# nvpro-samples/vk_gltf_renderer

Measured on AMD Instinct MI355X. Metric: Msamples/s (and ms/frame @ fixed spp) 1080p & 4K, 1/2/4/8 MI355X, higher is better.
Workload: dtype f32

## Files before the change

### vk_gltf_renderer_amd/csrc/device/mi_pt_api.hip

```cpp
#include <hip/hip_runtime.h>

#include <algorithm>
#include <chrono>
#include <cstdlib>
#include <cmath>
#include <cstdio>
#include <cstring>
#include <memory>
#include <string>
#include <vector>

#include "mi_pt.h"
#include "bvh_refit.h"
#include "material_patch.h"
#include "pt_build.h"
#include "pt_bvh.h"
#include "pt_deform.h"
#include "pt_kernels.h"

namespace {

thread_local std::string g_lastError;

int fail(int code, const std::string& msg)
// ... 129 lines not shown
  DevBuf<pt::DevPrim>         prims;
  DevBuf<MiGltfLight>         lights;
  DevBuf<pt::DevTexture>      textures;
  DevBuf<uchar4>              texels;
  DevBuf<uint4>               texQuads;
  DevBuf<uint8_t>             geometry;
  DevBuf<uint8_t>             instFlags;
  DevBuf<float>               srgbLut;
  DevBuf<float4>              envPixels;
  DevBuf<MiEnvAccel>          envAccel;
  DevBuf<pt::DevAlphaTri>     alphaTris;
  DevBuf<pt::DevShadeTri>     shadeTris;
  float4*                     bvhNodes  = nullptr;
  uint4*                      bvh8Nodes = nullptr;
  DevBuf<float>               bvh8Planes;
  pt::DevTri*                 bvhTris   = nullptr;
  bool                        wide      = true;
  pt::DevScene                scene{};
  bool                        hasAlpha = false, hasAlphaTest = false, hasVolumeScatter = false, simpleMaterials = true, hasTransmissive = false;
  static constexpr int        FC_RING = 32;
  DevBuf<pt::DevScene>        sceneDev;
  bool                        sceneDevDirty = true;
  DevBuf<pt::FrameConsts>     fcRing;
  DevBuf<pt::SkyPrecomp>      skyPre;
  MiSkyPhysicalParameters     skyPreFor{};
  bool                        skyPreValid = false;
  pt::FrameConsts*            fcHost = nullptr;
  hipEvent_t                  fcDone[FC_RING] = {};
  unsigned                    fcCursor = 0;
  MiPtStats                   staticStats{};
// ... 383 lines not shown
  }
  pt->lastUpdate = MI_PT_ACCEL_LAST_BUILD;
  if(rc != MI_PT_OK)
    dropAcceleration(pt);
  return rc;
}
void dropAcceleration(MiPt* pt)
{
  {
    const std::string why = g_lastError;
    releaseRefitData(pt);
    if(pt->bvhNodes) (void)hipFree(pt->bvhNodes);
    if(pt->bvhTris) (void)hipFree(pt->bvhTris);
    if(pt->bvh8Nodes) (void)hipFree(pt->bvh8Nodes);
    pt->bvhNodes = nullptr; pt->bvhTris = nullptr; pt->bvh8Nodes = nullptr;
    pt->bvh8Planes.release(); pt->shadeTris.release(); pt->alphaTris.release();
    pt::DevScene& S = pt->scene;
    S.bvhNodes = nullptr; S.bvh8Nodes = nullptr; S.tris = nullptr; S.bvh8Planes = nullptr; S.shadeTris = nullptr; S.alphaTris = nullptr;
    S.numTris = 0; S.bvh8NumNodes = 0; S.bvhRoot = pt::BVH_EMPTY;
    pt->staticStats.bvhNodeCount = pt->staticStats.bvhTriangleCount = 0;
    pt->sceneDevDirty = true;
    g_lastError = why;
  }
}
std::vector<uint8_t> instanceFlags(MiPt* pt)
{
  const int            numNodes = int(pt->hostNodes.size()), numMaterials = int(pt->matInstFlags.size());
  std::vector<uint8_t> flags(size_t(std::max(numNodes, 1)), 0);
  pt->hasAlpha = pt->hasAlphaTest = pt->hasTransmissive = pt->hasVolumeScatter = false;
  pt->simpleMaterials = true;
  for(int n = 0; n < numNodes; ++n)
  {
    const MiGltfRenderNode& rn = pt->hostNodes[size_t(n)];
// ... 136 lines not shown
      (void)hipFree(pt->bvhNodes);
      (void)hipFree(pt->bvhTris);
      pt->bvhNodes  = nullptr;
      pt->bvhTris   = b8.tris;
      pt->bvh8Nodes = b8.nodes;
      pt->scene.bvhRoot = 0;
      pt->scene.bvh8NumNodes = int(b8.numNodes);
      pt->staticStats.bvhNodeCount = b8.numNodes;
      pt->staticStats.bvhNodeBytes = 80;
      if(!pt->sw.noPlanes)
      {
        HIP_TRY(pt->bvh8Planes.alloc(size_t(b8.numNodes) * 48));
        pt::launchBvh8Planes(b8.nodes, b8.numNodes, pt->bvh8Planes.ptr, nullptr);
        HIP_TRY(hipGetLastError());
      }
      if(b8.slotBox && b8.nodeBox)
      {
        HIP_TRY(pt->refitBuiltBox.alloc(b8.numTris));
        HIP_TRY(hipMemcpy(pt->refitBuiltBox.ptr, b8.slotBox, sizeof(pt::RefitBox) * size_t(b8.numTris), hipMemcpyDeviceToDevice));
        HIP_TRY(pt->refitSah.alloc(b8.numNodes));
        HIP_TRY(pt->refitSahPartial.alloc(pt::REFIT_SAH_PARTIALS + 1));
        HIP_TRY(pt->refitDirty.alloc(std::max<size_t>(pt->hostNodes.size(), 1)));
        pt::launchRefitLevels(b8.nodes, b8.levels, pt->refitSlotBox.ptr, pt->refitNodeBox.ptr, pt->refitSah.ptr, nullptr);
        if(pt->bvh8Planes.ptr)
          pt::launchBvh8Planes(b8.nodes, b8.numNodes, pt->bvh8Planes.ptr, nullptr);
        HIP_TRY(hipGetLastError());
        if(int rc = readSahCost(pt, pt->sahAtBuild))
          return rc;
        pt->sahNow      = pt->sahAtBuild;
        pt->refitLevels = b8.levels;
        pt->builtNodes  = pt->hostNodes;
        pt->primDirty.assign(pt->primTriangles.size(), 0);
        pt->primDeformed.assign(pt->primTriangles.size(), 0);
        pt->residentTree = resident;
        pt->hiddenTris   = resident ? hiddenTris : 0;
      }
      else
      {
        pt->refitSlotBox.release();
        pt->refitNodeBox.release();
      }
    }
  }
  if(resident && !pt->residentTree && hiddenTris > 0)
  {
    --pt->accelBuilds;
    return buildAccelerationOver(pt, false);
  }
  pt::DevScene& S = pt->scene;
  S.bvhNodes = pt->bvhNodes; S.bvh8Nodes = pt->bvh8Nodes; S.tris = pt->bvhTris;
  S.bvh8Planes = pt->bvh8Nodes ? pt->bvh8Planes.ptr : nullptr;
  S.shadeTris = nullptr;
  S.alphaTris = nullptr;
  if(S.numTris > 0)
  {
    HIP_TRY(pt->shadeTris.alloc(size_t(S.numTris)));
    pt::launchBuildShadeRecords(S, uint32_t(S.numTris), pt->shadeTris.ptr, nullptr);
    HIP_TRY(hipGetLastError());
    HIP_TRY(hipDeviceSynchronize());
    S.shadeTris = pt->shadeTris.ptr;
  }
  if(pt->hasAlpha && S.numTris > 0)
  {
    HIP_TRY(pt->alphaTris.alloc(size_t(S.numTris)));
    pt::launchBuildAlphaRecords(S, uint32_t(S.numTris), pt->alphaTris.ptr, nullptr);
    HIP_TRY(hipGetLastError());
    HIP_TRY(hipDeviceSynchronize());
    S.alphaTris = pt->alphaTris.ptr;
  }
  if(pt->residentTree && pt->hiddenTris > 0)
  {
    std::vector<uint8_t> dirty(std::max<size_t>(pt->hostNodes.size(), 1), pt::REFIT_CLEAN);
    for(size_t n = 0; n < pt->hostNodes.size(); ++n)
      if(!pt->hostVisible[n])
        dirty[n] = pt::REFIT_HIDDEN;
    HIP_TRY(hipMemcpy(pt->refitDirty.ptr, dirty.data(), dirty.size(), hipMemcpyHostToDevice));
    pt::launchRefitTris(pt->nodes.ptr, pt->prims.ptr, pt->instFlags.ptr, pt->refitDirty.ptr, pt->refitBuiltBox.ptr, pt->bvhTris, pt->refitSlotBox.ptr,
                        uint32_t(S.numTris), nullptr);
    pt::launchRefitLevels(pt->bvh8Nodes, pt->refitLevels, pt->refitSlotBox.ptr, pt->refitNodeBox.ptr, pt->refitSah.ptr, nullptr);
    if(pt->bvh8Planes.ptr)
      pt::launchBvh8Planes(pt->bvh8Nodes, uint32_t(S.bvh8NumNodes), pt->bvh8Planes.ptr, nullptr);
    HIP_TRY(hipGetLastError());
    if(int rc = readSahCost(pt, pt->sahNow))
      return rc;
    HIP_TRY(hipDeviceSynchronize());
  }
  pt->sceneDevDirty = true;
  return MI_PT_OK;
}

int refitAcceleration(MiPt* pt, const std::vector<uint8_t>& moved, const std::vector<uint8_t>* visWas = nullptr)
{
  static const bool    buildTiming = getenv("MI_PT_BUILD_TIMING") != nullptr;
  const auto           t0          = std::chrono::steady_clock::now();
  const size_t         numNodes = pt->hostNodes.size(), numPrims = pt->primTriangles.size();
  std::vector<uint8_t> dirty(std::max<size_t>(numNodes, 1), pt::REFIT_CLEAN);
// ... 25 lines not shown
    const bool home = memcmp(rn.objectToWorld, pt->builtNodes[n].objectToWorld, sizeof(float) * 32) == 0 && !(ownsPrim && pt->primDeformed[size_t(rn.renderPrimID)]);
    dirty[n]        = home ? pt::REFIT_HOME : pt::REFIT_MOVED;
    if(ownsPrim && (pt->hostVisible.empty() || pt->hostVisible[n]))
      movedTris += pt->primTriangles[size_t(rn.renderPrimID)];
  }
  const std::vector<uint8_t> flags = instanceFlags(pt);
  const int                  rc    = [&]() -> int {
    HIP_TRY(hipMemcpy(pt->nodes.ptr, pt->hostNodes.data(), sizeof(MiGltfRenderNode) * numNodes, hipMemcpyHostToDevice));
    HIP_TRY(hipMemcpy(pt->instFlags.ptr, flags.data(), flags.size(), hipMemcpyHostToDevice));
    HIP_TRY(hipMemcpy(pt->refitDirty.ptr, dirty.data(), dirty.size(), hipMemcpyHostToDevice));
    pt::launchRefitTris(pt->nodes.ptr, pt->prims.ptr, pt->instFlags.ptr, pt->refitDirty.ptr, pt->refitBuiltBox.ptr, pt->bvhTris, pt->refitSlotBox.ptr,
                        uint32_t(pt->scene.numTris), nullptr);
    pt::launchRefitLevels(pt->bvh8Nodes, pt->refitLevels, pt->refitSlotBox.ptr, pt->refitNodeBox.ptr, pt->refitSah.ptr, nullptr);
    if(pt->bvh8Planes.ptr)
      pt::launchBvh8Planes(pt->bvh8Nodes, uint32_t(pt->scene.bvh8NumNodes), pt->bvh8Planes.ptr, nullptr);
    HIP_TRY(hipGetLastError());
    if(int e = readSahCost(pt, pt->sahNow))
      return e;
    HIP_TRY(hipDeviceSynchronize());
    return MI_PT_OK;
  }();
  if(rc != MI_PT_OK)
  {
    dropAcceleration(pt);
    return rc;
  }
  std::fill(pt->primDirty.begin(), pt->primDirty.end(), uint8_t(0));
  pt->sceneDevDirty = true;
  if(buildTiming)
    fprintf(stderr, "[mi_pt build] %-28s %8.2f ms\n", "refit", std::chrono::duration<double, std::milli>(std::chrono::steady_clock::now() - t0).count());
// ... 484 lines not shown
    HIP_TRY(pt->coreTex.upload(core.data(), core.size()));
  }
  {
    float lut[256];
    for(int i = 0; i < 256; ++i)
    {
      float c = float(i) / 255.0f;
      lut[i]  = c <= 0.04045f ? c / 12.92f : std::pow((c + 0.055f) / 1.055f, 2.4f);
    }
    HIP_TRY(pt->srgbLut.upload(lut, 256));
  }
  phase("textures upload");

  pt::DevScene& S = pt->scene;
  S.materials = pt->materials.ptr; S.texInfos = pt->texInfos.ptr; S.nodes = pt->nodes.ptr; S.prims = pt->prims.ptr; S.lights = pt->lights.ptr;
  S.textures = pt->textures.ptr; S.texels = pt->texels.ptr; S.texQuads = pt->texQuads.ptr; S.envPixels = nullptr; S.envAccel = nullptr; S.bvhNodes = nullptr; S.bvh8Nodes = nullptr; S.bvh8Planes = nullptr; S.tris = nullptr;
  S.geomPool = reinterpret_cast<const float4*>(pt->geometry.ptr);
  S.texRefs = pt->texRefs.ptr; S.coreTex = reinterpret_cast<const uint4*>(pt->coreTex.ptr); S.alphaTris = nullptr; S.shadeTris = nullptr; S.srgbLut = pt->srgbLut.ptr; S.numMaterials = sd->numMaterials; S.numTextures = sd->numTextures;
  S.numLights = sd->numLights; S.numNodes = sd->numRenderNodes;
  S.envWidth = 0; S.envHeight = 0;
  S.packetInterval = pt->sw.packetInterval;
  S.shadowOctFlip  = pt->sw.shadowFarFirst ? 7u : 0u;
  if(int rc = buildAcceleration(pt.get()))
    return rc;
  phase("shade / alpha records");
  HIP_TRY(pt->stats.alloc(1));
  HIP_TRY(hipMemset(pt->stats.ptr, 0, sizeof(pt::StatCounters)));
  MiSkyPhysicalParameters s{};
  s.rgbUnitConversion[0] = s.rgbUnitConversion[1] = s.rgbUnitConversion[2] = 1.0f / 80000.0f;
  s.multiplier = 0.1f; s.haze = 0.1f; s.redblueshift = 0.1f; s.saturation = 1.0f; s.groundColor[0] = s.groundColor[1] = s.groundColor[2] = 0.4f;
  s.horizonBlur = 0.3f; s.sunDiskIntensity = 1.0f; s.sunDirection[0] = s.sunDirection[1] = s.sunDirection[2] = 0.5773502691896258f;
// ... 1235 lines not shown

void* mi_pt_tonemapped_device_ptr(MiPt* pt)
{
  return pt ? pt->tonemapped.ptr : nullptr;
}

int mi_pt_get_memory(MiPt* pt, MiPtMemory* out)
{
  if(!pt || !out)
    return fail(MI_PT_ERR_ARGUMENT, "mi_pt_get_memory: null argument");
  HIP_TRY(hipSetDevice(pt->device));
  auto bytes = [](const auto& b) { return uint64_t(b.count) * sizeof(*b.ptr); };
  const pt::DevScene& sc = pt->scene;
  uint64_t scene = bytes(pt->materials) + bytes(pt->texInfos) + bytes(pt->nodes) + bytes(pt->prims) + bytes(pt->lights) + bytes(pt->textures) + bytes(pt->texels) + bytes(pt->texQuads)
                   + bytes(pt->geometry) + bytes(pt->instFlags) + bytes(pt->srgbLut) + bytes(pt->envPixels) + bytes(pt->envAccel) + bytes(pt->alphaTris)
                   + bytes(pt->shadeTris) + bytes(pt->texRefs) + bytes(pt->coreTex) + bytes(pt->bvh8Planes) + bytes(pt->deformPool) + bytes(pt->deformTasks)
                   + bytes(pt->deformBlockTask) + bytes(pt->deformJoints) + bytes(pt->deformWeights) + refitBytes(pt) + bytes(pt->vmPrevPositions) + bytes(pt->vmPrims)
                   + bytes(pt->vmDeformIDs);
  scene += uint64_t(pt->staticStats.bvhNodeCount) * pt->staticStats.bvhNodeBytes + uint64_t(sc.numTris) * sizeof(pt::DevTri);
  const uint64_t pathState = bytes(pt->pathArrays) + bytes(pt->optThroughput) + bytes(pt->optMisc) + bytes(pt->optMedium) + bytes(pt->optPixelSum) + bytes(pt->optGuides)
                             + bytes(pt->optShadowAux2) + bytes(pt->queueMem) + bytes(pt->queuePayload) + bytes(pt->candPool) + bytes(pt->candLists);
  const uint64_t renderer = pathState + bytes(pt->firstHit) + bytes(pt->accumOwn)
                            + bytes(pt->albedo) + bytes(pt->normal) + bytes(pt->denoiseA) + bytes(pt->denoiseB) + bytes(pt->tonemapped) + bytes(pt->depth)
                            + bytes(pt->selection) + bytes(pt->ownedTiles) + bytes(pt->sceneDev) + bytes(pt->fcRing) + bytes(pt->stats)
                            + bytes(pt->motion) + bytes(pt->history) + bytes(pt->prevObjectToWorld) + bytes(pt->firstHitTri);
  size_t freeB = 0, totalB = 0;
  HIP_TRY(hipMemGetInfo(&freeB, &totalB));
  out->sceneBytes       = scene;
  out->rendererBytes    = renderer;
  out->deviceUsedBytes  = uint64_t(totalB - freeB);
  out->deviceTotalBytes = uint64_t(totalB);
// ... 84 lines not shown
```

### vk_gltf_renderer_amd/csrc/device/pt_bvh8.h

```cpp
#pragma once
#include "pt_bvh.h"

namespace pt {

constexpr int BVH8_STACK_LDS  = MI_BVH8_STACK_LDS;
constexpr int BVH8_STACK_PRIV = 64 - MI_BVH8_STACK_LDS;

struct NodeGroup
{
  uint32_t base;
  uint32_t bits;
};

constexpr int WAIT_VMCNT0 = 0x0f70;

struct LaneStack2
{
  int*     lds;
  int      tid, stride;
  uint32_t *privBase, *privBits;
  int      sp;
  PT_DEV void push(NodeGroup g)
  {
    if(sp < BVH8_STACK_LDS)
// ... 114 lines not shown
    const float tn = fmaxf(fmaxf(tx.x, ty.x), fmaxf(tz.x, 0.0f));
    const float tf = fminf(fminf(tx.y, ty.y), fminf(tz.y, tmax));
    miss           = __builtin_amdgcn_alignbit(miss, __float_as_uint(tf - tn), 31);
  }
  const uint32_t hm = ~miss & 0xffu;
  uint32_t x = hm;
  x = (x | (x << 4)) & 0x0f0fu;
  x = (x | (x << 2)) & 0x3333u;
  x = (x | (x << 1)) & 0x5555u;
  x |= x << 1;
  const uint32_t valid = n1.z & 0xffffu;
  hmOut   = hm;
  leafOut = ((x & valid) << 16) | valid;
}

typedef float f32x8s __attribute__((ext_vector_type(8)));
PT_DEV uint32_t bvh8TestChildrenPlanes(const uint4& n0, const f32x8s& pnx, const f32x8s& pny, const f32x8s& pnz, const f32x8s& pfx, const f32x8s& pfy,
                                       const f32x8s& pfz, const RaySetup& r, float tmax, float sgnx, float sgny, float sgnz)
{
  const float sx = __uint_as_float((n0.w & 0xffu) << 23), sy = __uint_as_float(((n0.w >> 8) & 0xffu) << 23), sz = __uint_as_float(((n0.w >> 16) & 0xffu) << 23);
  const float Px = __uint_as_float(n0.x) - r.org.x, Py = __uint_as_float(n0.y) - r.org.y, Pz = __uint_as_float(n0.z) - r.org.z;
  const float Ax = sx * r.idir.x, Ay = sy * r.idir.y, Az = sz * r.idir.z;
  float       Bnx, Bfx, Bny, Bfy, Bnz, Bfz;
  (void)sgnx; (void)sgny; (void)sgnz;
  slabOffsets(Px, r.idir.x, Ax, Bnx, Bfx);
  slabOffsets(Py, r.idir.y, Ay, Bny, Bfy);
  slabOffsets(Pz, r.idir.z, Az, Bnz, Bfz);
  typedef float f32x2 __attribute__((ext_vector_type(2)));
  const f32x2 A2x = {Ax, Ax}, A2y = {Ay, Ay}, A2z = {Az, Az};
  const f32x2 Bn2x = {Bnx, Bnx}, Bn2y = {Bny, Bny}, Bn2z = {Bnz, Bnz}, Bf2x = {Bfx, Bfx}, Bf2y = {Bfy, Bfy}, Bf2z = {Bfz, Bfz};
// ... 4 lines not shown
    const int   i   = 6 - 2 * j;
    const f32x2 tnx = __builtin_elementwise_fma(f32x2{pnx[i], pnx[i + 1]}, A2x, Bn2x), tfx = __builtin_elementwise_fma(f32x2{pfx[i], pfx[i + 1]}, A2x, Bf2x);
    const f32x2 tny = __builtin_elementwise_fma(f32x2{pny[i], pny[i + 1]}, A2y, Bn2y), tfy = __builtin_elementwise_fma(f32x2{pfy[i], pfy[i + 1]}, A2y, Bf2y);
    const f32x2 tnz = __builtin_elementwise_fma(f32x2{pnz[i], pnz[i + 1]}, A2z, Bn2z), tfz = __builtin_elementwise_fma(f32x2{pfz[i], pfz[i + 1]}, A2z, Bf2z);
    const float tn1 = fmaxf(fmaxf(tnx.y, tny.y), fmaxf(tnz.y, 0.0f)), tf1 = fminf(fminf(tfx.y, tfy.y), fminf(tfz.y, tmax));
    miss            = __builtin_amdgcn_alignbit(miss, __float_as_uint(tf1 - tn1), 31);
    const float tn0 = fmaxf(fmaxf(tnx.x, tny.x), fmaxf(tnz.x, 0.0f)), tf0 = fminf(fminf(tfx.x, tfy.x), fminf(tfz.x, tmax));
    miss            = __builtin_amdgcn_alignbit(miss, __float_as_uint(tf0 - tn0), 31);
  }
  return ~miss & 0xffu;
}

PT_DEV void bvh8Visit(const DevScene& sc, const RaySetup& r, float tmax, uint32_t octinv, uint32_t nodeIndex, NodeGroup& outGroup, uint32_t& triBase,
                      uint32_t& leafWord, const uint4* ldsNodes, uint32_t cached, const uint8_t* octLut = nullptr)
{
  uint4 n0, n1, n2, n3, n4;
  if(nodeIndex < cached)
  {
    typedef uint32_t u32x4 __attribute__((ext_vector_type(4)));
    typedef const __attribute__((address_space(3))) u32x4* LdsNodePtr;
    LdsNodePtr  N = (LdsNodePtr)(ldsNodes) + nodeIndex * 5u;
    const u32x4 a = N[0], b = N[1], c = N[2], d = N[3], e = N[4];
    n0 = make_uint4(a[0], a[1], a[2], a[3]); n1 = make_uint4(b[0], b[1], b[2], b[3]); n2 = make_uint4(c[0], c[1], c[2], c[3]);
    n3 = make_uint4(d[0], d[1], d[2], d[3]); n4 = make_uint4(e[0], e[1], e[2], e[3]);
  }
  else
  {
    const uint4* N = sc.bvh8Nodes + size_t(nodeIndex) * 5;
    n0 = N[0]; n1 = N[1]; n2 = N[2]; n3 = N[3]; n4 = N[4];
  }
  const uint32_t imask = n0.w >> 24;
  uint32_t       hm, leaf;
  bvh8TestChildren(n0, n1, n2, n3, n4, r, tmax, hm, leaf);
  uint32_t hits = hm & imask;
  if(MI_PT_OCT_LUT && octLut)
  {
    typedef const __attribute__((address_space(3))) uint8_t* LdsBytePtr;
    hits = uint32_t(((LdsBytePtr)octLut)[(octinv << 8) | hits]);
  }
  else
    hits = octPermute(hits, octinv);
  outGroup.base = n1.x;
  outGroup.bits = (hits << 8) | imask;
  triBase       = n1.y;
  leafWord      = leaf;
}

}
// ... 1 lines not shown
```

### vk_gltf_renderer_amd/csrc/device/pt_kernels.h

```cpp
#pragma once
#include <hip/hip_runtime.h>

#include "pt_scene.h"
#include "pt_temporal.h"

namespace pt {

struct LaunchCtx
{
  DevScene        scene;
  FrameConsts     fc;
  const DevScene*    sceneDev;
  const FrameConsts* fcDev;
  PathSoA         paths;
  Queues          queues;
  const uint32_t* ownedTiles;
  StatCounters*   stats;
  hipStream_t     stream;
  unsigned        persistentBlocks;
  bool            hasAlpha;
  bool            hasAlphaClosest;
  bool            hasTransmissive;
  bool            simpleMaterials;
  bool            wide;
  bool            collectCounters;
  int             sortMode;
  bool            visualization;
};

void launchBuildShadeRecords(const DevScene& scene, uint32_t numTris, DevShadeTri* out, hipStream_t s);
void launchBuildAlphaRecords(const DevScene& scene, uint32_t numTris, DevAlphaTri* out, hipStream_t s);
void launchPatchMaterials(const DevScene& scene, const uint8_t* instFlags, const uint8_t* dirty, DevTri* tris, DevAlphaTri* alphaTris, DevShadeTri* shadeTris,
                          uint32_t numTris, hipStream_t s);
void dumpTraceProfile();
void launchBvh8Planes(const uint4* nodes, uint32_t numNodes, float* planes, hipStream_t s);
void launchTextureQuads(const uchar4* texels, uint4* quads, uint32_t offset, int width, int height, int wrapS, int wrapT, hipStream_t s);
void launchResetCounters(const Queues& Q, hipStream_t s);
void launchSkyPrecomp(const MiSkyPhysicalParameters& sky, SkyPrecomp* out, hipStream_t stream);
void launchGenerate(const LaunchCtx& c, int sampleIndex);
void launchTraceClosest(const LaunchCtx& c, int cur);
void launchTracePrimary(const LaunchCtx& c, int sampleIndex);
void launchShade(const LaunchCtx& c, int cur, bool first);
void launchTraceShadow(const LaunchCtx& c, int nxt);
void launchFlushSurvivors(const LaunchCtx& c, int cur);
void launchFinishSample(const LaunchCtx& c, int sampleIndex, float4* accum, float* depth, float4* albedo, float4* normal);
void launchSelection(const LaunchCtx& c, uint32_t* selection);

void launchAtrous(const float4* in, float4* out, const float4* albedo, const float4* normal, int width, int height, int step, float sigmaColor,
                  float sigmaNormal, float sigmaAlbedo, hipStream_t s);

// ... 19 lines not shown
```

### vk_gltf_renderer_amd/csrc/device/pt_kernels.hip

```cpp
#include <hip/hip_runtime.h>
#include <hip/hip_fp16.h>

#ifndef MI_PT_EXACT_FP
#define PT_FAST_SHADING_MATH 1
#endif
#include "pt_kernels.h"
#include "pt_shading.h"
#include "pt_bvh.h"
#include "pt_bvh8.h"
#include "pt_packet.h"
#include "pt_feed.h"
#include "pt_visualize.h"

namespace pt {

namespace {

constexpr int TRACE_BLOCK = 1024;
#ifndef NODE_CACHE_EXTRA
#define NODE_CACHE_EXTRA 0
#endif
constexpr int NODE_CACHE  = 712 + NODE_CACHE_EXTRA;
constexpr int NODE_CACHE_ALPHA = 504 + NODE_CACHE_EXTRA;
constexpr int SEL_BLOCK   = 256;
#ifndef TRACE_MIN_WAVES
#define TRACE_MIN_WAVES 1
#endif
constexpr int SHADE_BLOCK = 256;
constexpr uint32_t SORT_ROUNDS   = 4;
constexpr uint32_t SORT_WINDOW   = SORT_ROUNDS * SHADE_BLOCK;
constexpr uint32_t SORT_SEGMENTS = SORT_ROUNDS * (SHADE_BLOCK / 64);
constexpr int      SORT_BINS     = 32;
constexpr uint32_t SORT_BIN_MISS = 30;
constexpr uint32_t SORT_BIN_DEAD = 31;
#ifndef SHADE_SIMPLE_WAVES
#define SHADE_SIMPLE_WAVES 3
#endif

// ... 354 lines not shown
#endif
#ifndef TRI_ROUND_LANE_CAP_N
#define TRI_ROUND_LANE_CAP_N 4
#endif
constexpr int TRI_ROUND_LANE_CAP = TRI_ROUND_LANE_CAP_N;
#ifndef ALPHA_ROUND_MIN
#define ALPHA_ROUND_MIN 32
#endif
#ifndef ALPHA_ROUND_WAITING
#define ALPHA_ROUND_WAITING 8
#endif

PT_DEV uint32_t fillNodeCache(const DevScene& sc, uint4* s_nodes, uint32_t capacity = NODE_CACHE)
{
  const uint32_t n = min(uint32_t(sc.bvh8NumNodes), capacity);
  for(uint32_t i = threadIdx.x; i < n * 5u; i += blockDim.x)
    s_nodes[i] = sc.bvh8Nodes[i];
  __syncthreads();
  return n;
}

struct ClosestBest
{
  float    t, u, v;
  int      tri;
  uint32_t rnode, prim;
};
template <bool HAS_ALPHA>
PT_DEV void closestTestLoaded(const DevScene& sc, const RaySetup& r, const DevTri& T, int triIndex, ClosestBest& best, uint32_t& seed0, bool& seedLoaded,
                              const float4* misc, uint32_t slot);
template <bool HAS_ALPHA>
PT_DEV void closestTestTriangle(const DevScene& sc, const RaySetup& r, int triIndex, ClosestBest& best, uint32_t& seed0, bool& seedLoaded,
// ... 290 lines not shown
    ClosestBest none{};
    alphaDefer<true, REC>(sc, needAlpha, tr.item, ht, hu, hv, seed0, waveAlpha, aCount, aPending, none, occluded, rec);
    if(__ballot(needAlpha) & mine)
      aPending = true;
  }
  if(__ballot(commits) & mine)
    occluded = true;
}

template <bool WIDE, bool HAS_ALPHA, bool COUNT>
__global__ void __launch_bounds__(TRACE_BLOCK, TRACE_MIN_WAVES) k_trace_closest(DevScene sc, PathSoA P, Queues Q, int cur, StatCounters* stats)
{
  __shared__ int      s_stack[BVH_STACK_LDS * TRACE_BLOCK];
  __shared__ uint32_t s_prefix[NSUB + 1];
  constexpr int CACHE = HAS_ALPHA ? NODE_CACHE_ALPHA : NODE_CACHE;
  __shared__ uint4    s_nodes[WIDE ? CACHE * 5 : 1];
  __shared__ unsigned long long s_slots[WIDE ? TRACE_BLOCK : 1];
  __shared__ uint4    s_alpha[(WIDE && HAS_ALPHA) ? TRACE_BLOCK : 1];

  static_assert(2 * BVH8_STACK_LDS == BVH_STACK_LDS, "both stack flavours share one LDS allocation");
  if(blockIdx.x == 0 && threadIdx.x < NSUB)
  {
    Q.counters[(cur ? QC_PAIR0 : QC_PAIR1) + 2 * threadIdx.x]     = 0;
    Q.counters[(cur ? QC_PAIR0 : QC_PAIR1) + 2 * threadIdx.x + 1] = 0;
  }
  const RayQueue in = Q.active[cur];
  queuePrefix(&Q.counters[cur ? QC_PAIR1 : QC_PAIR0], s_prefix);
  WaveFeed feed;
  feedInit(feed, s_prefix[NSUB]);
  if(!feedBlockHasWork(feed))
    return;
// ... 605 lines not shown
{
  constexpr bool VIZ = false;
#include "pt_shade_body.h"
}
template <bool SIMPLE, bool FIRST>
__global__ void __launch_bounds__(SHADE_BLOCK, SIMPLE ? SHADE_SIMPLE_WAVES : 1) k_shade_viz(const DevScene* __restrict__ scp, const FrameConsts* __restrict__ fcp, PathSoA P, Queues Q, int cur, int sortMode, StatCounters* stats)
{
  constexpr bool COUNT = false, VIZ = true;
#include "pt_shade_body.h"
}

template <int MODE>
struct ShadowCfg
{
  static constexpr int BLOCK = MODE == 2 ? 256 : TRACE_BLOCK;
  static constexpr int CACHE = MODE == 2 ? 320 : (MODE == 1 ? NODE_CACHE_ALPHA : (MODE == 3 ? NODE_CACHE_ALPHA - 104 : NODE_CACHE));
};

PT_DEV void shadowDeposit(const PathSoA& P, const Queues& Q, int nxt, uint32_t slot, uint32_t qpos, bool catcherRay, f3 contrib, f3 total, bool occ,
                          float catcherDarken)
{
  if(!catcherRay)
  {
    if(!occ)
    {
      float4* const target = (slot & SHADOW_TARGET_QUEUE) ? &Q.active[nxt].rad[slot & ~SHADOW_TARGET_QUEUE] : &P.radiance[slot];
      float4        rad    = *target;
      rad.x += contrib.x * total.x;
      rad.y += contrib.y * total.y;
      rad.z += contrib.z * total.z;
      *target = rad;
// ... 17 lines not shown
    r3 -= contrib * (mk3(1.0f) - sf) * catcherDarken;
    rad.x = r3.x; rad.y = r3.y; rad.z = r3.z;
  }
  P.radiance[slot] = rad;
}

template <bool WIDE, int MODE, bool COUNT>
__global__ void __launch_bounds__(ShadowCfg<MODE>::BLOCK, TRACE_MIN_WAVES) k_trace_shadow(DevScene sc, const DevScene* __restrict__ scp, PathSoA P, Queues Q, int nxt, float catcherDarken, StatCounters* stats, int overflowOnly)
{
  constexpr int  SBLOCK    = ShadowCfg<MODE>::BLOCK;
  constexpr bool HAS_ALPHA = MODE >= 1, HAS_TRANS = MODE == 2, REC = MODE == 3;
  constexpr bool DEFER = MODE == 1 || MODE == 3;
  static_assert(!REC || WIDE, "the recording walk exists for the 8-wide BVH only");
  __shared__ int      s_stack[BVH_STACK_LDS * SBLOCK];
  __shared__ uint32_t s_prefix[NSUB + 1];
  __shared__ uint4    s_nodes[WIDE ? ShadowCfg<MODE>::CACHE * 5 : 1];
  __shared__ uint32_t s_items[(WIDE && !HAS_TRANS) ? SBLOCK : 1];
  __shared__ uint4    s_alpha[(WIDE && DEFER) ? SBLOCK : 1];
  __shared__ uint32_t s_head[REC ? SBLOCK : 1], s_ovf[REC ? SBLOCK : 1];
  __shared__ uint8_t  s_octLut[(WIDE && MI_PT_OCT_LUT) ? OCT_LUT_BYTES : 1];
  queuePrefix(&Q.counters[(nxt ? QC_PAIR1 : QC_PAIR0) + 1], s_prefix);
  const RayQueue in = Q.shadow;
  const bool     subset = MODE == 2 && overflowOnly != 0;
  uint32_t* const heads = &Q.counters[subset ? QC_HEADS_OVERFLOW : QC_HEADS_SHADOW];
  WaveFeed feed;
  feedInit(feed, subset ? Q.counters[QC_OVERFLOW] : s_prefix[NSUB]);
  if(!feedBlockHasWork(feed))
    return;
  if(WIDE && MI_PT_OCT_LUT)
    fillOctLut(s_octLut);
  const uint32_t cachedNodes = WIDE ? fillNodeCache(sc, s_nodes, uint32_t(ShadowCfg<MODE>::CACHE)) : 0u;
// ... 767 lines not shown
  const uint32_t id = blockIdx.x * 256u + threadIdx.x;
  if(id >= numNodes * 12u)
    return;
  const uint32_t  node = id / 12u, word = id % 12u;
  const uint32_t* rec  = reinterpret_cast<const uint32_t*>(nodes + size_t(node) * 5u) + 8u;
  const uint32_t  w    = rec[word];
  const uint32_t  pair = word >> 1, axis = pair % 3u, side = pair / 3u;
  float4          v    = make_float4(float(w & 0xffu), float((w >> 8) & 0xffu), float((w >> 16) & 0xffu), float(w >> 24));
  reinterpret_cast<float4*>(planes + size_t(node) * 48u + (2u * axis + side) * 8u)[word & 1u] = v;
}
void launchBvh8Planes(const uint4* nodes, uint32_t numNodes, float* planes, hipStream_t s)
{
  if(numNodes)
    hipLaunchKernelGGL(k_bvh8_planes, dim3((numNodes * 12u + 255u) / 256u), dim3(256), 0, s, nodes, numNodes, planes);
}
void launchTextureQuads(const uchar4* texels, uint4* quads, uint32_t offset, int width, int height, int wrapS, int wrapT, hipStream_t s)
{
  const uint32_t n = uint32_t(width) * uint32_t(height);
  hipLaunchKernelGGL(k_texture_quads, dim3((n + 255u) / 256u), dim3(256), 0, s, reinterpret_cast<const uint32_t*>(texels), quads, offset, width, height, wrapS, wrapT);
}
void launchResetCounters(const Queues& Q, hipStream_t s)
{
  hipLaunchKernelGGL(k_reset_counters, dim3(1), dim3(64), 0, s, Q.counters);
}
__global__ void k_sky_precomp(MiSkyPhysicalParameters sky, SkyPrecomp* out)
{
  if(blockIdx.x == 0 && threadIdx.x == 0)
    *out = makeSkyPrecomp(sky);
}
void launchSkyPrecomp(const MiSkyPhysicalParameters& sky, SkyPrecomp* out, hipStream_t stream)
// ... 155 lines not shown
```

### vk_gltf_renderer_amd/csrc/device/pt_scene.h

```cpp
#pragma once
#include <hip/hip_runtime.h>
#include <stdint.h>

#include "mi_pt.h"
#include "pt_math.h"

namespace pt {

struct DevTexture
{
  uint32_t levelOffset[16];
  uint16_t width, height;
  uint8_t  numLevels;
  uint8_t  srgb;
  uint8_t  magFilter, minFilter, mipmapMode, wrapS, wrapT;
  uint8_t  _pad[5];
};

struct DevTexRef
{
  float    uv[6];
  uint32_t level0;
  uint16_t width, height;
  uint8_t  numLevels, srgb, magFilter, minFilter, mipmapMode, wrapS, wrapT, texCoord;
// ... 89 lines not shown

struct DevScene
{
  const MiGltfShadeMaterial* materials;
  const MiGltfTextureInfo*   texInfos;
  const MiGltfRenderNode*    nodes;
  const DevPrim*             prims;
  const MiGltfLight*         lights;
  const DevTexture*          textures;
  const uchar4*              texels;
  const uint4*               texQuads;
  const float4*              envPixels;
  const MiEnvAccel*          envAccel;
  const float4*              bvhNodes;
  const uint4*               bvh8Nodes;
  const float*               bvh8Planes;
  const DevTri*              tris;
  const DevTexRef*           texRefs;
  const uint4*               coreTex;
  const DevShadeTri*         shadeTris;
  const float4*              geomPool;
  const DevAlphaTri*         alphaTris;
  const float*               srgbLut;
  int                        numMaterials, numTextures, numLights, numNodes;
  int                        envWidth, envHeight;
  int                        numTris;
  int                        bvh8NumNodes;
  int                        bvhRoot;
  int                        packetInterval;
  uint32_t                   shadowOctFlip;
// ... 167 lines not shown
```

Before: 751.2.

## Add 128-byte f16 walk-node layout for BVH8 traversal with sign-selected plane loads

Builds a second copy of each BVH8 node in a 128-byte layout where the quantized child bounds are pre-expanded to fp16 and grouped by axis and side. Traversal picks near/far plane offsets from the ray direction sign and loads only the needed halves, in two 4-child batches, from LDS or global memory. It also rebuilds this copy after every refit. The aim is to drop the per-node byte unpacking and the sign selects in the slab test. In exchange each node takes more space, so the LDS node cache holds 5/8 as many nodes and global traffic per node may rise.

```diff
diff --git a/vk_gltf_renderer_amd/csrc/device/mi_pt_api.hip b/vk_gltf_renderer_amd/csrc/device/mi_pt_api.hip
--- a/vk_gltf_renderer_amd/csrc/device/mi_pt_api.hip
+++ b/vk_gltf_renderer_amd/csrc/device/mi_pt_api.hip
@@ -167,6 +167,7 @@
   float4*                     bvhNodes  = nullptr;
   uint4*                      bvh8Nodes = nullptr;
   DevBuf<float>               bvh8Planes;
+  DevBuf<uint4>               bvh8WalkNodes;
   pt::DevTri*                 bvhTris   = nullptr;
   bool                        wide      = true;
   pt::DevScene                scene{};
@@ -580,9 +581,9 @@
     if(pt->bvhTris) (void)hipFree(pt->bvhTris);
     if(pt->bvh8Nodes) (void)hipFree(pt->bvh8Nodes);
     pt->bvhNodes = nullptr; pt->bvhTris = nullptr; pt->bvh8Nodes = nullptr;
-    pt->bvh8Planes.release(); pt->shadeTris.release(); pt->alphaTris.release();
+    pt->bvh8Planes.release(); pt->bvh8WalkNodes.release(); pt->shadeTris.release(); pt->alphaTris.release();
     pt::DevScene& S = pt->scene;
-    S.bvhNodes = nullptr; S.bvh8Nodes = nullptr; S.tris = nullptr; S.bvh8Planes = nullptr; S.shadeTris = nullptr; S.alphaTris = nullptr;
+    S.bvhNodes = nullptr; S.bvh8Nodes = nullptr; S.tris = nullptr; S.bvh8Planes = nullptr; S.bvh8WalkNodes = nullptr; S.shadeTris = nullptr; S.alphaTris = nullptr;
     S.numTris = 0; S.bvh8NumNodes = 0; S.bvhRoot = pt::BVH_EMPTY;
     pt->staticStats.bvhNodeCount = pt->staticStats.bvhTriangleCount = 0;
     pt->sceneDevDirty = true;
@@ -749,6 +750,14 @@
         pt::launchBvh8Planes(b8.nodes, b8.numNodes, pt->bvh8Planes.ptr, nullptr);
         HIP_TRY(hipGetLastError());
       }
+      if(pt::walkNodesInUse())
+      {
+        if(b8.numNodes > (1u << 25))
+          return fail(MI_PT_ERR_HIP, "BVH8 has more than 2^25 nodes");
+        HIP_TRY(pt->bvh8WalkNodes.alloc(size_t(b8.numNodes) * 8));
+        pt::launchBvh8WalkNodes(b8.nodes, b8.numNodes, pt->bvh8WalkNodes.ptr, nullptr);
+        HIP_TRY(hipGetLastError());
+      }
       if(b8.slotBox && b8.nodeBox)
       {
         HIP_TRY(pt->refitBuiltBox.alloc(b8.numTris));
@@ -759,6 +768,7 @@
         pt::launchRefitLevels(b8.nodes, b8.levels, pt->refitSlotBox.ptr, pt->refitNodeBox.ptr, pt->refitSah.ptr, nullptr);
         if(pt->bvh8Planes.ptr)
           pt::launchBvh8Planes(b8.nodes, b8.numNodes, pt->bvh8Planes.ptr, nullptr);
+        pt::launchBvh8WalkNodes(b8.nodes, b8.numNodes, pt->bvh8WalkNodes.ptr, nullptr);
         HIP_TRY(hipGetLastError());
         if(int rc = readSahCost(pt, pt->sahAtBuild))
           return rc;
@@ -785,6 +795,7 @@
   pt::DevScene& S = pt->scene;
   S.bvhNodes = pt->bvhNodes; S.bvh8Nodes = pt->bvh8Nodes; S.tris = pt->bvhTris;
   S.bvh8Planes = pt->bvh8Nodes ? pt->bvh8Planes.ptr : nullptr;
+  S.bvh8WalkNodes = pt->bvh8Nodes ? pt->bvh8WalkNodes.ptr : nullptr;
   S.shadeTris = nullptr;
   S.alphaTris = nullptr;
   if(S.numTris > 0)
@@ -815,6 +826,7 @@
     pt::launchRefitLevels(pt->bvh8Nodes, pt->refitLevels, pt->refitSlotBox.ptr, pt->refitNodeBox.ptr, pt->refitSah.ptr, nullptr);
     if(pt->bvh8Planes.ptr)
       pt::launchBvh8Planes(pt->bvh8Nodes, uint32_t(S.bvh8NumNodes), pt->bvh8Planes.ptr, nullptr);
+    pt::launchBvh8WalkNodes(pt->bvh8Nodes, uint32_t(S.bvh8NumNodes), pt->bvh8WalkNodes.ptr, nullptr);
     HIP_TRY(hipGetLastError());
     if(int rc = readSahCost(pt, pt->sahNow))
       return rc;
@@ -870,6 +882,7 @@
     pt::launchRefitLevels(pt->bvh8Nodes, pt->refitLevels, pt->refitSlotBox.ptr, pt->refitNodeBox.ptr, pt->refitSah.ptr, nullptr);
     if(pt->bvh8Planes.ptr)
       pt::launchBvh8Planes(pt->bvh8Nodes, uint32_t(pt->scene.bvh8NumNodes), pt->bvh8Planes.ptr, nullptr);
+    pt::launchBvh8WalkNodes(pt->bvh8Nodes, uint32_t(pt->scene.bvh8NumNodes), pt->bvh8WalkNodes.ptr, nullptr);
     HIP_TRY(hipGetLastError());
     if(int e = readSahCost(pt, pt->sahNow))
       return e;
@@ -1384,7 +1397,7 @@
 
   pt::DevScene& S = pt->scene;
   S.materials = pt->materials.ptr; S.texInfos = pt->texInfos.ptr; S.nodes = pt->nodes.ptr; S.prims = pt->prims.ptr; S.lights = pt->lights.ptr;
-  S.textures = pt->textures.ptr; S.texels = pt->texels.ptr; S.texQuads = pt->texQuads.ptr; S.envPixels = nullptr; S.envAccel = nullptr; S.bvhNodes = nullptr; S.bvh8Nodes = nullptr; S.bvh8Planes = nullptr; S.tris = nullptr;
+  S.textures = pt->textures.ptr; S.texels = pt->texels.ptr; S.texQuads = pt->texQuads.ptr; S.envPixels = nullptr; S.envAccel = nullptr; S.bvhNodes = nullptr; S.bvh8Nodes = nullptr; S.bvh8WalkNodes = nullptr; S.bvh8Planes = nullptr; S.tris = nullptr;
   S.geomPool = reinterpret_cast<const float4*>(pt->geometry.ptr);
   S.texRefs = pt->texRefs.ptr; S.coreTex = reinterpret_cast<const uint4*>(pt->coreTex.ptr); S.alphaTris = nullptr; S.shadeTris = nullptr; S.srgbLut = pt->srgbLut.ptr; S.numMaterials = sd->numMaterials; S.numTextures = sd->numTextures;
   S.numLights = sd->numLights; S.numNodes = sd->numRenderNodes;
@@ -2650,7 +2663,7 @@
   const pt::DevScene& sc = pt->scene;
   uint64_t scene = bytes(pt->materials) + bytes(pt->texInfos) + bytes(pt->nodes) + bytes(pt->prims) + bytes(pt->lights) + bytes(pt->textures) + bytes(pt->texels) + bytes(pt->texQuads)
                    + bytes(pt->geometry) + bytes(pt->instFlags) + bytes(pt->srgbLut) + bytes(pt->envPixels) + bytes(pt->envAccel) + bytes(pt->alphaTris)
-                   + bytes(pt->shadeTris) + bytes(pt->texRefs) + bytes(pt->coreTex) + bytes(pt->bvh8Planes) + bytes(pt->deformPool) + bytes(pt->deformTasks)
+                   + bytes(pt->shadeTris) + bytes(pt->texRefs) + bytes(pt->coreTex) + bytes(pt->bvh8Planes) + bytes(pt->bvh8WalkNodes) + bytes(pt->deformPool) + bytes(pt->deformTasks)
                    + bytes(pt->deformBlockTask) + bytes(pt->deformJoints) + bytes(pt->deformWeights) + refitBytes(pt) + bytes(pt->vmPrevPositions) + bytes(pt->vmPrims)
                    + bytes(pt->vmDeformIDs);
   scene += uint64_t(pt->staticStats.bvhNodeCount) * pt->staticStats.bvhNodeBytes + uint64_t(sc.numTris) * sizeof(pt::DevTri);
diff --git a/vk_gltf_renderer_amd/csrc/device/pt_bvh8.h b/vk_gltf_renderer_amd/csrc/device/pt_bvh8.h
--- a/vk_gltf_renderer_amd/csrc/device/pt_bvh8.h
+++ b/vk_gltf_renderer_amd/csrc/device/pt_bvh8.h
@@ -1,5 +1,10 @@
 #pragma once
 #include "pt_bvh.h"
+#include "walk_node.h"
+
+#ifndef MI_PT_WALK_F16
+#define MI_PT_WALK_F16 1
+#endif
 
 namespace pt {
 
@@ -152,6 +157,87 @@
   leafOut = ((x & valid) << 16) | valid;
 }
 
+PT_DEV float halfLo(uint32_t w)
+{
+  typedef _Float16 f16x2 __attribute__((ext_vector_type(2)));
+  return float(__builtin_bit_cast(f16x2, w)[0]);
+}
+PT_DEV float halfHi(uint32_t w)
+{
+  typedef _Float16 f16x2 __attribute__((ext_vector_type(2)));
+  return float(__builtin_bit_cast(f16x2, w)[1]);
+}
+struct SlabCoeffs
+{
+  float Ax, Ay, Az, Bnx, Bny, Bnz, Bfx, Bfy, Bfz;
+};
+PT_DEV SlabCoeffs slabCoeffs(const uint4& n0, const RaySetup& r)
+{
+  const float sx = __uint_as_float((n0.w & 0xffu) << 23), sy = __uint_as_float(((n0.w >> 8) & 0xffu) << 23), sz = __uint_as_float(((n0.w >> 16) & 0xffu) << 23);
+  const float Px = __uint_as_float(n0.x) - r.org.x, Py = __uint_as_float(n0.y) - r.org.y, Pz = __uint_as_float(n0.z) - r.org.z;
+  SlabCoeffs  c;
+  c.Ax = sx * r.idir.x; c.Ay = sy * r.idir.y; c.Az = sz * r.idir.z;
+  slabOffsets(Px, r.idir.x, c.Ax, c.Bnx, c.Bfx);
+  slabOffsets(Py, r.idir.y, c.Ay, c.Bny, c.Bfy);
+  slabOffsets(Pz, r.idir.z, c.Az, c.Bnz, c.Bfz);
+  return c;
+}
+PT_DEV uint32_t slabTest4F16(uint32_t miss, const uint2& nearX, const uint2& nearY, const uint2& nearZ, const uint2& farX, const uint2& farY, const uint2& farZ,
+                             const SlabCoeffs& c, float tmax)
+{
+#pragma unroll
+  for(int j = 0; j < 4; ++j)
+  {
+    const int   i  = 3 - j;
+    const bool  hi = i & 1, up = i >> 1;
+    const uint32_t qnx = up ? nearX.y : nearX.x, qny = up ? nearY.y : nearY.x, qnz = up ? nearZ.y : nearZ.x;
+    const uint32_t qfx = up ? farX.y : farX.x, qfy = up ? farY.y : farY.x, qfz = up ? farZ.y : farZ.x;
+    const float tnx = __fmaf_rn(hi ? halfHi(qnx) : halfLo(qnx), c.Ax, c.Bnx), tfx = __fmaf_rn(hi ? halfHi(qfx) : halfLo(qfx), c.Ax, c.Bfx);
+    const float tny = __fmaf_rn(hi ? halfHi(qny) : halfLo(qny), c.Ay, c.Bny), tfy = __fmaf_rn(hi ? halfHi(qfy) : halfLo(qfy), c.Ay, c.Bfy);
+    const float tnz = __fmaf_rn(hi ? halfHi(qnz) : halfLo(qnz), c.Az, c.Bnz), tfz = __fmaf_rn(hi ? halfHi(qfz) : halfLo(qfz), c.Az, c.Bfz);
+    const float tn  = fmaxf(fmaxf(tnx, tny), fmaxf(tnz, 0.0f));
+    const float tf  = fminf(fminf(tfx, tfy), fminf(tfz, tmax));
+    miss            = __builtin_amdgcn_alignbit(miss, __float_as_uint(tf - tn), 31);
+  }
+  return miss;
+}
+PT_DEV void slabResult(uint32_t miss, uint32_t valid16, uint32_t& hmOut, uint32_t& leafOut)
+{
+  const uint32_t hm = ~miss & 0xffu;
+  uint32_t x = hm;
+  x = (x | (x << 4)) & 0x0f0fu;
+  x = (x | (x << 2)) & 0x3333u;
+  x = (x | (x << 1)) & 0x5555u;
+  x |= x << 1;
+  const uint32_t valid = valid16 & 0xffffu;
+  hmOut   = hm;
+  leafOut = ((x & valid) << 16) | valid;
+}
+PT_DEV void bvh8TestChildrenF16(const uint4& n0, const uint4& n1, const uint4& nearX, const uint4& nearY, const uint4& nearZ, const uint4& farX, const uint4& farY,
+                                const uint4& farZ, const RaySetup& r, float tmax, uint32_t& hmOut, uint32_t& leafOut)
+{
+  const SlabCoeffs c = slabCoeffs(n0, r);
+  uint32_t miss = slabTest4F16(0u, make_uint2(nearX.z, nearX.w), make_uint2(nearY.z, nearY.w), make_uint2(nearZ.z, nearZ.w), make_uint2(farX.z, farX.w),
+                               make_uint2(farY.z, farY.w), make_uint2(farZ.z, farZ.w), c, tmax);
+  miss = slabTest4F16(miss, make_uint2(nearX.x, nearX.y), make_uint2(nearY.x, nearY.y), make_uint2(nearZ.x, nearZ.y), make_uint2(farX.x, farX.y),
+                      make_uint2(farY.x, farY.y), make_uint2(farZ.x, farZ.y), c, tmax);
+  slabResult(miss, n1.z, hmOut, leafOut);
+}
+
+struct WalkOffsets
+{
+  uint32_t nearX, nearY, nearZ;
+};
+PT_DEV WalkOffsets walkNodeOffsets(f3 idir)
+{
+  WalkOffsets o;
+  o.nearX = idir.x < 0.0f ? 80u : 32u;
+  o.nearY = idir.y < 0.0f ? 96u : 48u;
+  o.nearZ = idir.z < 0.0f ? 112u : 64u;
+  return o;
+}
+constexpr uint32_t WALK_FAR_XOR_X = 32u ^ 80u, WALK_FAR_XOR_Y = 48u ^ 96u, WALK_FAR_XOR_Z = 64u ^ 112u;
+
 typedef float f32x8s __attribute__((ext_vector_type(8)));
 PT_DEV uint32_t bvh8TestChildrenPlanes(const uint4& n0, const f32x8s& pnx, const f32x8s& pny, const f32x8s& pnz, const f32x8s& pfx, const f32x8s& pfy,
                                        const f32x8s& pfz, const RaySetup& r, float tmax, float sgnx, float sgny, float sgnz)
@@ -186,11 +272,54 @@
 PT_DEV void bvh8Visit(const DevScene& sc, const RaySetup& r, float tmax, uint32_t octinv, uint32_t nodeIndex, NodeGroup& outGroup, uint32_t& triBase,
                       uint32_t& leafWord, const uint4* ldsNodes, uint32_t cached, const uint8_t* octLut = nullptr)
 {
+  typedef uint32_t u32x4 __attribute__((ext_vector_type(4)));
+  typedef const __attribute__((address_space(3))) u32x4* LdsNodePtr;
+  uint32_t hm, leaf;
+#if MI_PT_WALK_F16
+  typedef const __attribute__((address_space(3))) char* LdsBytePtr0;
+  const WalkOffsets o    = walkNodeOffsets(r.idir);
+  const uint32_t    base = nodeIndex * WALK_NODE_BYTES;
+  const uint32_t    aNx = base + o.nearX, aNy = base + o.nearY, aNz = base + o.nearZ;
+  const uint32_t    aFx = aNx ^ WALK_FAR_XOR_X, aFy = aNy ^ WALK_FAR_XOR_Y, aFz = aNz ^ WALK_FAR_XOR_Z;
+  typedef uint32_t u32x2 __attribute__((ext_vector_type(2)));
+  typedef const __attribute__((address_space(3))) u32x2* LdsHalfPtr;
+  uint4 n0, n1;
+  uint2 pnx, pny, pnz, pfx, pfy, pfz;
+  const bool fromLds = nodeIndex < cached;
+  const LdsBytePtr0 L = (LdsBytePtr0)(ldsNodes);
+  const char*       W = reinterpret_cast<const char*>(sc.bvh8WalkNodes);
+  if(fromLds)
+  {
+    const LdsNodePtr N = (LdsNodePtr)(L + base);
+    const u32x4 a = N[0], b = N[1]; const u32x2 c = *(LdsHalfPtr)(L + aNx + 8u), d = *(LdsHalfPtr)(L + aNy + 8u), e = *(LdsHalfPtr)(L + aNz + 8u), f = *(LdsHalfPtr)(L + aFx + 8u), g = *(LdsHalfPtr)(L + aFy + 8u), h = *(LdsHalfPtr)(L + aFz + 8u);
+    n0 = make_uint4(a[0], a[1], a[2], a[3]); n1 = make_uint4(b[0], b[1], b[2], b[3]);
+    pnx = make_uint2(c[0], c[1]); pny = make_uint2(d[0], d[1]); pnz = make_uint2(e[0], e[1]); pfx = make_uint2(f[0], f[1]); pfy = make_uint2(g[0], g[1]); pfz = make_uint2(h[0], h[1]);
+  }
+  else
+  {
+    const uint4* N = reinterpret_cast<const uint4*>(W + base);
+    n0 = N[0]; n1 = N[1]; pnx = *reinterpret_cast<const uint2*>(W + aNx + 8u); pny = *reinterpret_cast<const uint2*>(W + aNy + 8u); pnz = *reinterpret_cast<const uint2*>(W + aNz + 8u); pfx = *reinterpret_cast<const uint2*>(W + aFx + 8u); pfy = *reinterpret_cast<const uint2*>(W + aFy + 8u); pfz = *reinterpret_cast<const uint2*>(W + aFz + 8u);
+  }
+  const SlabCoeffs co = slabCoeffs(n0, r);
+  uint32_t miss = slabTest4F16(0u, pnx, pny, pnz, pfx, pfy, pfz, co, tmax);
+#ifndef MI_PT_WALK_F16_UPFRONT
+  asm volatile("" : "+v"(miss) : : "memory");
+#endif
+  if(fromLds)
+  {
+    const u32x2 c = *(LdsHalfPtr)(L + aNx), d = *(LdsHalfPtr)(L + aNy), e = *(LdsHalfPtr)(L + aNz), f = *(LdsHalfPtr)(L + aFx), g = *(LdsHalfPtr)(L + aFy), h = *(LdsHalfPtr)(L + aFz);
+    pnx = make_uint2(c[0], c[1]); pny = make_uint2(d[0], d[1]); pnz = make_uint2(e[0], e[1]); pfx = make_uint2(f[0], f[1]); pfy = make_uint2(g[0], g[1]); pfz = make_uint2(h[0], h[1]);
+  }
+  else
+  {
+    pnx = *reinterpret_cast<const uint2*>(W + aNx); pny = *reinterpret_cast<const uint2*>(W + aNy); pnz = *reinterpret_cast<const uint2*>(W + aNz); pfx = *reinterpret_cast<const uint2*>(W + aFx); pfy = *reinterpret_cast<const uint2*>(W + aFy); pfz = *reinterpret_cast<const uint2*>(W + aFz);
+  }
+  miss = slabTest4F16(miss, pnx, pny, pnz, pfx, pfy, pfz, co, tmax);
+  slabResult(miss, n1.z, hm, leaf);
+#else
   uint4 n0, n1, n2, n3, n4;
   if(nodeIndex < cached)
   {
-    typedef uint32_t u32x4 __attribute__((ext_vector_type(4)));
-    typedef const __attribute__((address_space(3))) u32x4* LdsNodePtr;
     LdsNodePtr  N = (LdsNodePtr)(ldsNodes) + nodeIndex * 5u;
     const u32x4 a = N[0], b = N[1], c = N[2], d = N[3], e = N[4];
     n0 = make_uint4(a[0], a[1], a[2], a[3]); n1 = make_uint4(b[0], b[1], b[2], b[3]); n2 = make_uint4(c[0], c[1], c[2], c[3]);
@@ -201,9 +330,9 @@
     const uint4* N = sc.bvh8Nodes + size_t(nodeIndex) * 5;
     n0 = N[0]; n1 = N[1]; n2 = N[2]; n3 = N[3]; n4 = N[4];
   }
+  bvh8TestChildren(n0, n1, n2, n3, n4, r, tmax, hm, leaf);
+#endif
   const uint32_t imask = n0.w >> 24;
-  uint32_t       hm, leaf;
-  bvh8TestChildren(n0, n1, n2, n3, n4, r, tmax, hm, leaf);
   uint32_t hits = hm & imask;
   if(MI_PT_OCT_LUT && octLut)
   {
diff --git a/vk_gltf_renderer_amd/csrc/device/pt_kernels.h b/vk_gltf_renderer_amd/csrc/device/pt_kernels.h
--- a/vk_gltf_renderer_amd/csrc/device/pt_kernels.h
+++ b/vk_gltf_renderer_amd/csrc/device/pt_kernels.h
@@ -34,6 +34,8 @@
                           uint32_t numTris, hipStream_t s);
 void dumpTraceProfile();
 void launchBvh8Planes(const uint4* nodes, uint32_t numNodes, float* planes, hipStream_t s);
+bool walkNodesInUse();
+void launchBvh8WalkNodes(const uint4* nodes, uint32_t numNodes, uint4* walk, hipStream_t s);
 void launchTextureQuads(const uchar4* texels, uint4* quads, uint32_t offset, int width, int height, int wrapS, int wrapT, hipStream_t s);
 void launchResetCounters(const Queues& Q, hipStream_t s);
 void launchSkyPrecomp(const MiSkyPhysicalParameters& sky, SkyPrecomp* out, hipStream_t stream);
diff --git a/vk_gltf_renderer_amd/csrc/device/pt_kernels.hip b/vk_gltf_renderer_amd/csrc/device/pt_kernels.hip
--- a/vk_gltf_renderer_amd/csrc/device/pt_kernels.hip
+++ b/vk_gltf_renderer_amd/csrc/device/pt_kernels.hip
@@ -20,8 +20,10 @@
 #ifndef NODE_CACHE_EXTRA
 #define NODE_CACHE_EXTRA 0
 #endif
-constexpr int NODE_CACHE  = 712 + NODE_CACHE_EXTRA;
-constexpr int NODE_CACHE_ALPHA = 504 + NODE_CACHE_EXTRA;
+constexpr int NODE_UINT4 = MI_PT_WALK_F16 ? 8 : 5;
+constexpr int nodeCacheFor(int records80) { return MI_PT_WALK_F16 ? records80 * 5 / 8 : records80; }
+constexpr int NODE_CACHE  = nodeCacheFor(712 + NODE_CACHE_EXTRA);
+constexpr int NODE_CACHE_ALPHA = nodeCacheFor(504 + NODE_CACHE_EXTRA);
 constexpr int SEL_BLOCK   = 256;
 #ifndef TRACE_MIN_WAVES
 #define TRACE_MIN_WAVES 1
@@ -406,8 +408,9 @@
 PT_DEV uint32_t fillNodeCache(const DevScene& sc, uint4* s_nodes, uint32_t capacity = NODE_CACHE)
 {
   const uint32_t n = min(uint32_t(sc.bvh8NumNodes), capacity);
-  for(uint32_t i = threadIdx.x; i < n * 5u; i += blockDim.x)
-    s_nodes[i] = sc.bvh8Nodes[i];
+  const uint4* src = MI_PT_WALK_F16 ? sc.bvh8WalkNodes : sc.bvh8Nodes;
+  for(uint32_t i = threadIdx.x; i < n * uint32_t(NODE_UINT4); i += blockDim.x)
+    s_nodes[i] = src[i];
   __syncthreads();
   return n;
 }
@@ -728,7 +731,7 @@
   __shared__ int      s_stack[BVH_STACK_LDS * TRACE_BLOCK];
   __shared__ uint32_t s_prefix[NSUB + 1];
   constexpr int CACHE = HAS_ALPHA ? NODE_CACHE_ALPHA : NODE_CACHE;
-  __shared__ uint4    s_nodes[WIDE ? CACHE * 5 : 1];
+  __shared__ uint4    s_nodes[WIDE ? CACHE * NODE_UINT4 : 1];
   __shared__ unsigned long long s_slots[WIDE ? TRACE_BLOCK : 1];
   __shared__ uint4    s_alpha[(WIDE && HAS_ALPHA) ? TRACE_BLOCK : 1];
 
@@ -1364,7 +1367,7 @@
 struct ShadowCfg
 {
   static constexpr int BLOCK = MODE == 2 ? 256 : TRACE_BLOCK;
-  static constexpr int CACHE = MODE == 2 ? 320 : (MODE == 1 ? NODE_CACHE_ALPHA : (MODE == 3 ? NODE_CACHE_ALPHA - 104 : NODE_CACHE));
+  static constexpr int CACHE = MODE == 2 ? nodeCacheFor(320) : (MODE == 1 ? NODE_CACHE_ALPHA : (MODE == 3 ? nodeCacheFor(504 + NODE_CACHE_EXTRA - 104) : NODE_CACHE));
 };
 
 PT_DEV void shadowDeposit(const PathSoA& P, const Queues& Q, int nxt, uint32_t slot, uint32_t qpos, bool catcherRay, f3 contrib, f3 total, bool occ,
@@ -1412,7 +1415,7 @@
   static_assert(!REC || WIDE, "the recording walk exists for the 8-wide BVH only");
   __shared__ int      s_stack[BVH_STACK_LDS * SBLOCK];
   __shared__ uint32_t s_prefix[NSUB + 1];
-  __shared__ uint4    s_nodes[WIDE ? ShadowCfg<MODE>::CACHE * 5 : 1];
+  __shared__ uint4    s_nodes[WIDE ? ShadowCfg<MODE>::CACHE * NODE_UINT4 : 1];
   __shared__ uint32_t s_items[(WIDE && !HAS_TRANS) ? SBLOCK : 1];
   __shared__ uint4    s_alpha[(WIDE && DEFER) ? SBLOCK : 1];
   __shared__ uint32_t s_head[REC ? SBLOCK : 1], s_ovf[REC ? SBLOCK : 1];
@@ -2210,6 +2213,31 @@
   if(numNodes)
     hipLaunchKernelGGL(k_bvh8_planes, dim3((numNodes * 12u + 255u) / 256u), dim3(256), 0, s, nodes, numNodes, planes);
 }
+__global__ void __launch_bounds__(256) k_bvh8_walk_nodes(const uint4* __restrict__ nodes, uint32_t numNodes, uint4* __restrict__ walk)
+{
+  const uint32_t id = blockIdx.x * 256u + threadIdx.x;
+  if(id >= numNodes * 8u)
+    return;
+  const uint32_t node = id >> 3, part = id & 7u;
+  const uint4*   rec  = nodes + size_t(node) * 5u;
+  uint4          out;
+  if(part < 2u)
+    out = rec[part];
+  else
+  {
+    const uint32_t* q = reinterpret_cast<const uint32_t*>(rec) + 8u + 2u * (part - 2u);
+    uint32_t        w[4];
+    walkNodeBlock(q[0], q[1], w);
+    out = make_uint4(w[0], w[1], w[2], w[3]);
+  }
+  walk[size_t(id)] = out;
+}
+bool walkNodesInUse() { return MI_PT_WALK_F16 != 0; }
+void launchBvh8WalkNodes(const uint4* nodes, uint32_t numNodes, uint4* walk, hipStream_t s)
+{
+  if(numNodes && walk)
+    hipLaunchKernelGGL(k_bvh8_walk_nodes, dim3((numNodes * 8u + 255u) / 256u), dim3(256), 0, s, nodes, numNodes, walk);
+}
 void launchTextureQuads(const uchar4* texels, uint4* quads, uint32_t offset, int width, int height, int wrapS, int wrapT, hipStream_t s)
 {
   const uint32_t n = uint32_t(width) * uint32_t(height);
diff --git a/vk_gltf_renderer_amd/csrc/device/pt_scene.h b/vk_gltf_renderer_amd/csrc/device/pt_scene.h
--- a/vk_gltf_renderer_amd/csrc/device/pt_scene.h
+++ b/vk_gltf_renderer_amd/csrc/device/pt_scene.h
@@ -127,6 +127,7 @@
   const MiEnvAccel*          envAccel;
   const float4*              bvhNodes;
   const uint4*               bvh8Nodes;
+  const uint4*               bvh8WalkNodes;
   const float*               bvh8Planes;
   const DevTri*              tris;
   const DevTexRef*           texRefs;
diff --git a/vk_gltf_renderer_amd/csrc/device/walk_node.h b/vk_gltf_renderer_amd/csrc/device/walk_node.h
--- /dev/null
+++ b/vk_gltf_renderer_amd/csrc/device/walk_node.h
@@ -0,0 +1,53 @@
+#pragma once
+#include "bvh_refit.h"
+
+namespace pt {
+
+struct WalkNode8
+{
+  uint32_t head0[4];
+  uint32_t head1[4];
+  uint16_t plane[6][8];
+};
+static_assert(sizeof(WalkNode8) == 128, "WalkNode8 must be 128 bytes");
+
+constexpr uint32_t WALK_NODE_BYTES       = 128;
+constexpr uint32_t WALK_NODE_PLANES_BYTE = 32;
+
+PT_DEV uint16_t walkHalfOfByte(uint32_t q)
+{
+  if(q == 0u)
+    return 0;
+  uint32_t e = 0;
+  for(uint32_t v = q; v > 1u; v >>= 1)
+    ++e;
+  return uint16_t(((e + 15u) << 10) | ((q << (10u - e)) & 0x3ffu));
+}
+
+PT_DEV void walkNodeBlock(uint32_t q0123, uint32_t q4567, uint32_t (&out)[4])
+{
+  for(int w = 0; w < 4; ++w)
+  {
+    const uint32_t src = w < 2 ? q0123 : q4567, sh = 16u * uint32_t(w & 1);
+    out[w] = uint32_t(walkHalfOfByte((src >> sh) & 0xffu)) | (uint32_t(walkHalfOfByte((src >> (sh + 8u)) & 0xffu)) << 16);
+  }
+}
+
+PT_DEV void walkNodeFromNode8(const Node8& N, WalkNode8& W)
+{
+  __builtin_memcpy(W.head0, &N, 16);
+  __builtin_memcpy(W.head1, reinterpret_cast<const char*>(&N) + 16, 16);
+  for(uint32_t b = 0; b < 6u; ++b)
+  {
+    uint32_t w[4], q[2];
+    __builtin_memcpy(q, b < 3u ? N.qlo[b] : N.qhi[b - 3u], 8);
+    walkNodeBlock(q[0], q[1], w);
+    for(int i = 0; i < 4; ++i)
+    {
+      W.plane[b][2 * i]     = uint16_t(w[i] & 0xffffu);
+      W.plane[b][2 * i + 1] = uint16_t(w[i] >> 16);
+    }
+  }
+}
+
+}
```

Result: slower. 691.7 (-7.9%).
